# Dimitrinov74/Domain-Specific-Image-Compression

Hardware: AMD Instinct MI355X
Metric: 256x256 satellite patches encoded/s per GPU; bpp + MS-SSIM vs reference (higher is better)
Workload: dtype f32 (Winograd contractions as split-bf16 MFMA with fp32 accumulate); 1 GPU; batch=64/GPU 256x256x3 synthetic patches, modelv2 encode->decode (g_a,h_a,round,h_s,Student-t/Gaussian rate,g_s) + bpp + MS-SSIM[.3,.5,.2] on GPU + CDF tables and range coder (z,y strings) on GPU [BASELINE config 3]; global_batch=64, parallelism=per-image sharding x1, one all-reduce of 4 fp64, weights=synthetic seed 1 (checkpoints absent from the reference)

## Files before the change

### domain-specific-image-compression_amd/csrc/conv_wino_bf16.h

```cpp
#pragma once
#include <stdlib.h>

#include <type_traits>

#include "common.h"

#ifndef WB_PLANES
#define WB_PLANES 2
#endif
#ifndef WB_STAMP
#define WB_STAMP 0
#endif
#ifndef WB_ABL
#define WB_ABL 0
#endif
#ifndef WB_ADOUBLE
#define WB_ADOUBLE 0
#endif
#ifndef WB_HPRIO
#define WB_HPRIO 3
#endif
#ifndef WB_STAMP_TILE
#define WB_STAMP_TILE 8
#endif
// ... 19 lines not shown
  const float* beta;
  const float* gamma;
  float* out;
  int B, H, W, Cin, Cout, CoutP;
  int act;
  unsigned long long* ticket;
  int nphase;
  int64_t u_phase_bytes;
  int s2d_in, s2d;
  int tiles_x, tiles_y, ntiles;
  int nt_out;
  int ostride, ooff;
  int ksplit, kchunks;
  int64_t part_stride;
  int cm_in, cm_out;
};

constexpr int P = WB_PLANES;
constexpr int CK = 16;
constexpr int ROWB = CK * 2;
constexpr int POSB = 32 * ROWB;
constexpr int PLANEB = 16 * POSB;
constexpr int VBUFB = P * PLANEB;
constexpr int WP = 36;
constexpr int YOFF = 2 * VBUFB;
constexpr int YBYTES = 16 * 32 * WP * 4;
constexpr int SLOTOFF = YOFF + YBYTES;
constexpr int WINW = 18, WINH = 10;
constexpr int WINB = WINW * WINH * CK * 4;
constexpr int STAGEOFF = SLOTOFF + 64;
// ... 82 lines not shown
```

### domain-specific-image-compression_amd/csrc/conv_wino_bf16m.hip

```cpp
#include "conv_wino_bf16.h"

#ifndef WBM_STAMP
#define WBM_STAMP 0
#endif
#ifndef WBM_ABL
#define WBM_ABL 0
#endif

namespace dsic {
namespace wbm {

using wb::Args;
using wb::bf16_hi;
using wb::bf16_lo;
using wb::bf16x8;
using wb::cvt_pk_bf16;
using wb::floatx16;
using wb::floatx2;
using wb::floatx4;
using wb::intx4;
using wb::Tile;
using wb::uintx2;
using wb::uintx4;

// ... 2 lines not shown
constexpr int NTILE = 64;
constexpr int ROWB = CK * 2;
constexpr int POSB = NTILE * ROWB;
constexpr int PLANEB = 8 * POSB;
constexpr int VBUFB = P * PLANEB;
constexpr int XOFF = 2 * VBUFB;
constexpr int XBYTES = 8 * 4096;
constexpr int SLOTOFF = XOFF + XBYTES;
constexpr int WINW = 18, WINH = 18;
constexpr int WINITEMS = WINW * WINH * 4;
constexpr int WINB = WINITEMS * 16;
constexpr int NLOAD = (WINITEMS + 255) / 256;
constexpr int STAGEOFF = SLOTOFF + 64;
constexpr int NWIN = 3;
constexpr int STAMPOFF = STAGEOFF + NWIN * WINB;
constexpr int PARAMOFF = STAMPOFF + (WBM_STAMP ? 1024 : 0);
constexpr int LDS_TOTAL = PARAMOFF + 3 * 128 * 4;
constexpr int THREADS = 768;
constexpr int RING = 2;

static_assert(LDS_TOTAL <= 160 * 1024, "LDS budget");

#if WBM_STAMP
static __device__ long long wbm_stamps[256 * 256];
#define MSTAMP(w, i)                                                                                   \
  do {                                                                                                 \
    __builtin_amdgcn_sched_barrier(0);                                                                 \
    if (lane == 0 && wave == (w) && tile_count == 3 && (i) >= 0 && (i) < 128)                          \
      ((unsigned*)(lds_raw + STAMPOFF))[((w) == 0 ? 0 : 128) + (i)] = (unsigned)__builtin_amdgcn_s_memtime();   \
    __builtin_amdgcn_sched_barrier(0);                                                                 \
  } while (0)
#else
#define MSTAMP(w, i)
#endif

__device__ __forceinline__ int lane_now() {
  int l;
  asm volatile("v_mbcnt_lo_u32_b32 %0, -1, 0\n\tv_mbcnt_hi_u32_b32 %0, -1, %0" : "=v"(l));
  return l;
}

template <int MODE, int PASS, int PQ>
struct Steps {
  static constexpr unsigned value =
      PASS == 0 ? (PQ == 0 ? (MODE == 2 ? 0x4567u : 0x7654u) : (MODE == 2 ? 0x89ABu : 0xBA98u))
                : (PQ == 0 ? (MODE == 2 ? 0x0123u : 0x3210u) : (MODE == 2 ? 0xCDEFu : 0xFEDCu));
};
template <int MODE, int PASS, int PQ>
__device__ __forceinline__ constexpr int gpos(int s) {
  return (int)((Steps<MODE, PASS, PQ>::value >> (4 * s)) & 15u);
}
template <int PASS>
__device__ __forceinline__ constexpr int lpos_of(int g) {
  return PASS == 0 ? ((g >> 2) - 1) * 4 + (g & 3) : ((g >> 2) == 3 ? 4 : 0) + (g & 3);
}
template <int MODE, int PASS, int PQ>
__device__ __forceinline__ constexpr int step_of(int g) {
  for (int s = 0; s < 4; ++s)
    if (gpos<MODE, PASS, PQ>(s) == g) return s;
  return -1;
}

template <int MODE, bool NT_OUT>
__global__ __launch_bounds__(THREADS) void conv_wino_bf16m_kernel(const Args a) {
  extern __shared__ __attribute__((aligned(16))) unsigned char lds_raw[];
  float* const slots = (float*)(lds_raw + SLOTOFF);
  const int tid = threadIdx.x, lane = tid & 63;
  const int wave = __builtin_amdgcn_readfirstlane(tid >> 6);
  auto read_slot = [&](int s) {
    const intx4 v = *(const intx4*)(slots + 4 * s);
    Tile t;
    t.item = __builtin_amdgcn_readfirstlane(v[0]);
    t.tx = __builtin_amdgcn_readfirstlane(v[1]);
    t.ty = __builtin_amdgcn_readfirstlane(v[2]);
    t.n = __builtin_amdgcn_readfirstlane(v[3]);
    t.ks = 0;
    return t;
  };
  const int pshift = a.nphase == 4 ? 2 : 0;
  const int nchunks = a.Cin / CK;
  const int L = 2 * nchunks;
  int tile_count = 0;
  (void)tile_count;
  if (tid < 128) {
    float* const prm = (float*)(lds_raw + PARAMOFF);
    const bool cv = tid < a.Cout, gd = cv && (a.act == DSIC_ACT_GDN || a.act == DSIC_ACT_IGDN);
    prm[tid] = cv ? a.bias[tid] : 0.f;
    prm[128 + tid] = gd ? a.beta[tid] : 1.f;
    prm[256 + tid] = gd ? a.gamma[tid] : 0.f;
  }

  if (wave >= 8) {
    __builtin_amdgcn_s_setprio(3);
    const int ht = tid - 512;
    const int Cin = a.Cin;
    const int pt = ht >> 2, pq = ht & 3;
// ... 1 lines not shown
    const int vwrite = pt * ROWB + ((((pq >> 1) ^ ((pt >> 3) & 1))) << 4) + ((pq & 1) << 3);
    unsigned char* const vmine = lds_raw + vwrite;
    auto post = [&](int s, int item) {
      const int tile = item >> pshift;
      const int row = tile / a.tiles_x;
      const intx4 v = {item, tile - row * a.tiles_x, row % a.tiles_y, row / a.tiles_y};
      *(intx4*)(slots + 4 * s) = v;
    };
    const int pix_f = a.cm_in ? CK : Cin;
    const unsigned chunk_in_b = a.cm_in ? (unsigned)(a.H * a.W * CK * 4) : (unsigned)(CK * 4);
    struct WinAim {
      unsigned off[NLOAD];
      uintx4 rsrc;
    };
    WinAim am;
    const int hw = wave - 8;
    const unsigned lds_base = (unsigned)(unsigned long long)(__attribute__((address_space(3))) unsigned char*)lds_raw;
    auto aim = [&](WinAim& m, const Tile& t0) {
      Tile t = t0;
      if (WBM_ABL & 1) { t.n = 0; t.tx = 0; t.ty = 0; }
      const unsigned long long base = (unsigned long long)(a.in + (size_t)t.n * a.H * a.W * Cin);
      m.rsrc = uintx4{(unsigned)base, (unsigned)(base >> 32) & 0xFFFFu, (unsigned)(a.H * a.W * Cin * 4), 0x00020000u};
#pragma unroll
      for (int j = 0; j < NLOAD; ++j) {
        const int i = ht + 256 * j;
        const int pix = i >> 2, q = i & 3;
        const int wy = pix / WINW, wx = pix - wy * WINW;
        const int gy = t.ty * 16 - 1 + wy, gx = t.tx * 16 - 1 + wx;
        const bool ok = i < WINITEMS && gy >= 0 && gy < a.H && gx >= 0 && gx < a.W && !(WBM_ABL & 2);
        m.off[j] = ok ? (unsigned)(((gy * a.W + gx) * pix_f + 4 * q) * 4) : 0x80000000u;
      }
    };
    auto aim_nowhere = [&](WinAim& m) {
#pragma unroll
      for (int j = 0; j < NLOAD; ++j) m.off[j] = 0x80000000u;
    };
    auto dma = [&](int wbuf, int chunk) {
      const uintx4 rs = {(unsigned)__builtin_amdgcn_readfirstlane((int)am.rsrc[0]), (unsigned)__builtin_amdgcn_readfirstlane((int)am.rsrc[1]),
                         (unsigned)__builtin_amdgcn_readfirstlane((int)am.rsrc[2]), (unsigned)__builtin_amdgcn_readfirstlane((int)am.rsrc[3])};
      const unsigned soff = (unsigned)chunk * chunk_in_b;
#pragma unroll
      for (int j = 0; j < NLOAD; ++j) {
        const unsigned m0v = lds_base + (unsigned)(STAGEOFF + wbuf * WINB + 16 * (hw * 64 + 256 * j));
        if (j < NLOAD - 1 || ht < WINITEMS - 256 * (NLOAD - 1))
          asm volatile("s_mov_b32 m0, %0\n\ts_nop 0\n\tbuffer_load_dwordx4 %1, %2, %3 offen lds"
                       :: "s"(m0v), "v"(am.off[j]), "s"(rs), "s"(soff) : "memory");
      }
    };
    const bool last_piece = hw == 0;
    auto wait_all_but_newest = [&](int groups) {
      if (groups == 0) asm volatile("s_waitcnt vmcnt(0)" ::: "memory");
      else if (groups == 1) { if (last_piece) asm volatile("s_waitcnt vmcnt(6)" ::: "memory"); else asm volatile("s_waitcnt vmcnt(5)" ::: "memory"); }
      else { if (last_piece) asm volatile("s_waitcnt vmcnt(12)" ::: "memory"); else asm volatile("s_waitcnt vmcnt(10)" ::: "memory"); }
    };
    static_assert(NLOAD == 6, "the vmcnt immediates above count 6 (5) loads per window");
    const int patch0 = ((2 * pty) * WINW + 2 * ptx) * (CK * 4) + pq * 16;
    auto psub = [](floatx2 x, floatx2 y) {
      floatx2 r;
      asm("v_pk_add_f32 %0, %1, %2 neg_lo:[0,1] neg_hi:[0,1]" : "=v"(r) : "v"(x), "v"(y));
      return r;
    };
    auto sub4 = [&](floatx4 x, floatx4 y) {
      const floatx2 l = psub(floatx2{x[0], x[1]}, floatx2{y[0], y[1]}), h = psub(floatx2{x[2], x[3]}, floatx2{y[2], y[3]});
      return floatx4{l[0], l[1], h[0], h[1]};
    };
    auto split_store = [&](floatx4 v, unsigned char* dst) {
      const unsigned h0 = cvt_pk_bf16(v[0], v[1]), h1 = cvt_pk_bf16(v[2], v[3]);
      *(uintx2*)dst = uintx2{h0, h1};
      const floatx2 r01 = psub(floatx2{v[0], v[1]}, floatx2{bf16_lo(h0), bf16_hi(h0)});
      const floatx2 r23 = psub(floatx2{v[2], v[3]}, floatx2{bf16_lo(h1), bf16_hi(h1)});
// ... 3 lines not shown
      const unsigned char* src = lds_raw + STAGEOFF + wbuf * WINB + patch0;
      unsigned char* dst = vmine + vb * VBUFB;
      floatx4 xa[4], xb[4];
      bool a_live = true, b_live = true;
      if (!passB) {
#pragma unroll
        for (int k = 0; k < 4; ++k) {
          const floatx4 r1 = *(const floatx4*)(src + (1 * WINW + k) * (CK * 4));
          const floatx4 r2 = *(const floatx4*)(src + (2 * WINW + k) * (CK * 4));
          xa[k] = r1 + r2;
          xb[k] = sub4(r2, r1);
        }
      } else {
        a_live = zxi != 0u;
        b_live = zxi != 3u;
#pragma unroll
        for (int k = 0; k < 4; ++k) {
          const floatx4 r0 = *(const floatx4*)(src + (0 * WINW + k) * (CK * 4));
          const floatx4 r1 = *(const floatx4*)(src + (1 * WINW + k) * (CK * 4));
          const floatx4 r2 = *(const floatx4*)(src + (2 * WINW + k) * (CK * 4));
          const floatx4 r3 = *(const floatx4*)(src + (3 * WINW + k) * (CK * 4));
          xa[k] = sub4(r0, r2);
          xb[k] = sub4(r1, r3);
        }
      }
      if (a_live) {
        if (znu != 0) split_store(sub4(xa[0], xa[2]), dst + 0 * POSB);
        split_store(xa[1] + xa[2], dst + 1 * POSB);
        split_store(sub4(xa[2], xa[1]), dst + 2 * POSB);
        if (znu != 3) split_store(sub4(xa[1], xa[3]), dst + 3 * POSB);
      }
      if (b_live) {
        if (znu != 0) split_store(sub4(xb[0], xb[2]), dst + 4 * POSB);
        split_store(xb[1] + xb[2], dst + 5 * POSB);
        split_store(sub4(xb[2], xb[1]), dst + 6 * POSB);
        if (znu != 3) split_store(sub4(xb[1], xb[3]), dst + 7 * POSB);
      }
    };
    auto zero_of = [&](const Tile& t, int k, unsigned& zxi, unsigned& znu) {
      zxi = 4;
      znu = 4;
      if (MODE == 1) {
        const int blk = k / (nchunks >> 2);
        if (blk >> 1) zxi = 3;
        if (blk & 1) znu = 3;
      } else if (MODE == 2) {
        const int phase = t.item & 3;
        if (phase >> 1) zxi = 0;
        if (phase & 1) znu = 0;
      }
    };
    auto next_ticket = [&]() { return (int)(atomicAdd(a.ticket, 1ULL) + gridDim.x); };

    if (ht == 0) {
      post(0, (int)blockIdx.x);
      post(1, next_ticket());
    }
    __syncthreads();
    Tile cur = read_slot(0);
    int ticket_pre = a.ntiles;
    aim(am, cur);
    dma(0, 0);
    dma(1, 1);
    dma(2, 2);
    if (ht == 0 && read_slot(1).item < a.ntiles) ticket_pre = next_ticket();
    wait_all_but_newest(2);
    __syncthreads();
    {
      unsigned zxi, znu;
      zero_of(cur, 0, zxi, znu);
      commit(0, 0, false, zxi, znu);
    }
    wait_all_but_newest(1);
    __syncthreads();
    int wq = 1;
    int s_nxt = 1, s_wr = 2;
    while (cur.item < a.ntiles) {
      const Tile nxt = read_slot(s_nxt);
      const bool more = nxt.item < a.ntiles;
      tile_count++;
      auto phase = [&](int sg) {
        MSTAMP(8, 4 * sg);
        {
          const int k3 = sg + 3;
          if (k3 == L) {
            if (more) aim(am, nxt); else aim_nowhere(am);
          }
          const int k3w = k3 < L ? k3 : k3 - L;
          dma(wq >= 1 ? wq - 1 : 2, k3w < nchunks ? k3w : k3w - nchunks);
        }
        MSTAMP(8, 4 * sg + 1);
        {
          unsigned zxi, znu;
          const int tg = sg + 1;
          const bool passB = tg >= nchunks && tg < L;
          if (tg < L) zero_of(cur, passB ? tg - nchunks : tg, zxi, znu); else zero_of(nxt, 0, zxi, znu);
          commit(wq, tg & 1, passB, zxi, znu);
        }
        wq = wq == 2 ? 0 : wq + 1;
        wait_all_but_newest(1);
        MSTAMP(8, 4 * sg + 2);
        __syncthreads();
        MSTAMP(8, 4 * sg + 3);
      };
      if (ht == 0 && more) post(s_wr, ticket_pre);
      for (int sg = 0; sg < L; sg += 2) {
        phase(sg);
        phase(sg + 1);
        if (sg + 2 == nchunks) {
          __syncthreads();
          __syncthreads();
          __syncthreads();
          __syncthreads();
        }
      }
      if (ht == 0 && more && read_slot(s_wr).item < a.ntiles) ticket_pre = next_ticket();
      cur = nxt;
      const int s_old = s_nxt;
      s_nxt = s_wr;
      s_wr = s_old == 0 ? 2 : s_old - 1;
    }
#if WBM_STAMP
    if (wave == 8) {
      wbm_stamps[blockIdx.x * 256 + 128 + lane] = (long long)((unsigned*)(lds_raw + STAMPOFF))[128 + lane];
      wbm_stamps[blockIdx.x * 256 + 192 + lane] = (long long)((unsigned*)(lds_raw + STAMPOFF))[192 + lane];
    }
#endif
    if (ht == 0) {
      const unsigned long long done = atomicAdd(a.ticket + 1, 1ULL);
      if (done == (unsigned long long)gridDim.x - 1) {
        a.ticket[0] = 0ULL;
        a.ticket[1] = 0ULL;
      }
    }
    return;
  }

  const int h = lane >> 5, l31 = lane & 31;
  const int nt = wave & 3, pqw = wave >> 2;
  const bool nvalid = nt * 32 < a.CoutP;
// ... 50 lines not shown
  Tile cur = read_slot(0);
  const __amdgpu_buffer_rsrc_t urs = __builtin_amdgcn_make_buffer_rsrc(
      (void*)a.u, 0, (int)(16u * pos_b * (unsigned)a.nphase), 0x00020000);
  auto soff_item = [&](const Tile& t) { return (unsigned)(t.item & (a.nphase - 1)) * (unsigned)a.u_phase_bytes; };
  unsigned soff_phase = soff_item(cur);
  auto fetch = [&](bf16x8 (&dst)[P], unsigned so) {
#pragma unroll
    for (int q = 0; q < P; ++q)
      dst[q] = __builtin_bit_cast(bf16x8, __builtin_amdgcn_raw_buffer_load_b128(urs, ulane, so + (unsigned)q * plane_b, 0));
  };
#pragma unroll
  for (int f = 0; f < RING; ++f) fetch(Bq[f], soff_phase + (unsigned)gpos<MODE, 0, PQ>(f) * pos_b);
  int s_nxt = 1;
  while (cur.item < a.ntiles) {
    tile_count++;
    const Tile nxt = read_slot(s_nxt);
    const unsigned soff_phase_nxt = soff_item(nxt.item < a.ntiles ? nxt : cur);
    unsigned tzero_xi = 4, tzero_nu = 4;
    if (MODE == 2) {
      const int phase = cur.item & 3;
      if (phase >> 1) tzero_xi = 0;
      if (phase & 1) tzero_nu = 0;
    }
    auto chunk_body = [&](auto pass_tag, auto first_tag, int chunk) {
      constexpr int PASS = decltype(pass_tag)::value;
      constexpr bool FIRST = decltype(first_tag)::value;
      const bool last = chunk + 1 == nchunks;
      MSTAMP(0, 3 * (PASS * nchunks + chunk));
      unsigned zero_xi = tzero_xi, zero_nu = tzero_nu;
      if (MODE == 1) {
        const int blk = chunk / (nchunks >> 2);
        zero_xi = (blk >> 1) ? 3 : 4;
        zero_nu = (blk & 1) ? 3 : 4;
      }
      auto is_zero = [&](int s) {
        const int g = gpos<MODE, PASS, PQ>(s);
        return (unsigned)(g >> 2) == zero_xi || (unsigned)(g & 3) == zero_nu;
      };
      const unsigned char* vb = lds_raw + ((PASS * nchunks + chunk) & 1) * VBUFB + aread;
      auto vaddr = [&](int sub, int q) {
        return vb + lpos_of<PASS>(gpos<MODE, PASS, PQ>(sub >> 1)) * POSB + (sub & 1) * (32 * ROWB) + q * PLANEB;
      };
      bf16x8 Aq[P];
#pragma unroll
      for (int q = 0; q < P; ++q) Aq[q] = *(const bf16x8*)vaddr(0, q);
#pragma unroll
      for (int s = 0; s < 4; ++s) {
        const bool live = !ZSKIP || !is_zero(s);
// ... 11 lines not shown
#pragma unroll
            for (int e = 0; e < 16; ++e) acc[sub][e] = 0.f;
          }
          if (sub + 1 < 8) {
#pragma unroll
            for (int q = 0; q < P; ++q) Aq[q] = *(const bf16x8*)vaddr(sub + 1, q);
          }
        }
        {
          const int f = s + RING;
          const unsigned so = f < 4 ? soff_phase + (unsigned)gpos<MODE, PASS, PQ>(f) * pos_b + (unsigned)chunk * chunk_b
                                    : soff_phase + (unsigned)gpos<MODE, PASS, PQ>(f - 4) * pos_b + (unsigned)(chunk + 1) * chunk_b;
          if (f < 4 ? !(ZSKIP && is_zero(f)) : !last) fetch(Bq[s % RING], so);
        }
      }
      MSTAMP(0, 3 * (PASS * nchunks + chunk) + 1);
      __syncthreads();
      MSTAMP(0, 3 * (PASS * nchunks + chunk) + 2);
    };

    chunk_body(std::integral_constant<int, 0>{}, std::true_type{}, 0);
    for (int chunk = 1; chunk < nchunks; ++chunk) chunk_body(std::integral_constant<int, 0>{}, std::false_type{}, chunk);
    {
      constexpr int XI = 1 + PQ;
      constexpr int s0 = step_of<MODE, 0, PQ>(XI * 4 + 0), s1 = step_of<MODE, 0, PQ>(XI * 4 + 1);
      constexpr int s2 = step_of<MODE, 0, PQ>(XI * 4 + 2), s3 = step_of<MODE, 0, PQ>(XI * 4 + 3);
      floatx16 c0[2], c1[2];
#pragma unroll
      for (int m = 0; m < 2; ++m) {
        c0[m] = (acc[2 * s0 + m] + acc[2 * s1 + m]) + acc[2 * s2 + m];
        c1[m] = (acc[2 * s1 + m] - acc[2 * s2 + m]) - acc[2 * s3 + m];
      }
      constexpr int XB = PQ == 0 ? 0 : 3;
      constexpr int t0 = step_of<MODE, 1, PQ>(XB * 4 + 0), t1 = step_of<MODE, 1, PQ>(XB * 4 + 1);
      constexpr int t2 = step_of<MODE, 1, PQ>(XB * 4 + 2), t3 = step_of<MODE, 1, PQ>(XB * 4 + 3);
#pragma unroll
      for (int m = 0; m < 2; ++m) {
        xwrite(xa_mine, c0[m]);
        xwrite(xb_mine, c1[m]);
        MSTAMP(0, 122 + 2 * m);
        __syncthreads();
        MSTAMP(0, 123 + 2 * m);
        const floatx16 g0 = xread(xa_part), g1 = xread(xb_part);
        if (PQ == 0) {
          acc[2 * t0 + m] = c0[m] + g0;
          acc[2 * t3 + m] = -(c1[m] + g1);
        } else {
          acc[2 * t0 + m] = c0[m] - g0;
          acc[2 * t3 + m] = g1 - c1[m];
        }
#pragma unroll
        for (int e = 0; e < 16; ++e) {
          acc[2 * t1 + m][e] = 0.f;
          acc[2 * t2 + m][e] = 0.f;
        }
        __syncthreads();
      }
      MSTAMP(0, 126);
    }
#pragma unroll
    for (int f = 0; f < RING; ++f) fetch(Bq[f], soff_phase + (unsigned)gpos<MODE, 1, PQ>(f) * pos_b);
    for (int chunk = 0; chunk < nchunks; ++chunk) chunk_body(std::integral_constant<int, 1>{}, std::false_type{}, chunk);
    soff_phase = soff_phase_nxt;

    MSTAMP(0, 120);
    {
      const int phase = cur.item & (a.nphase - 1);
      const int ppy = phase >> 1, ppx = phase & 1;
      const int OH = a.nphase == 4 ? 2 * a.H : a.H, OW = a.nphase == 4 ? 2 * a.W : a.W;
      const __amdgpu_buffer_rsrc_t ors = __builtin_amdgcn_make_buffer_rsrc(
          (void*)(a.out + (size_t)cur.n * OH * OW * a.ostride + a.ooff), 0, (OH * OW * a.ostride - a.ooff) * 4, 0x00020000);
      const unsigned tbase =
          a.nphase == 4 ? (unsigned)(((32 * cur.ty + ppy) * OW + 32 * cur.tx + ppx) * PB)
          : a.s2d       ? (unsigned)(((8 * cur.ty) * (a.W >> 1) + 8 * cur.tx) * SX)
                        : (unsigned)((16 * cur.ty * a.W + 16 * cur.tx) * PB);
      constexpr int XB = PQ == 0 ? 0 : 3;
      constexpr int t0 = step_of<MODE, 1, PQ>(XB * 4 + 0), t1 = step_of<MODE, 1, PQ>(XB * 4 + 1);
      constexpr int t2 = step_of<MODE, 1, PQ>(XB * 4 + 2), t3 = step_of<MODE, 1, PQ>(XB * 4 + 3);
      const int ln = lane_now();
      float* const tw = (float*)(lds_raw + XOFF + wave * 4096) + ln + 96 * (ln >> 5);
// ... 36 lines not shown
        else if (a.act == DSIC_ACT_IGDN)
          emit(std::integral_constant<int, DSIC_ACT_IGDN>{}, m, j, y);
        else if (a.act == DSIC_ACT_RELU)
          emit(std::integral_constant<int, DSIC_ACT_RELU>{}, m, j, y);
        else
          emit(std::integral_constant<int, DSIC_ACT_NONE>{}, m, j, y);
      };
#pragma unroll
      for (int m = 0; m < 2; ++m) {
        const floatx16 y0 = (acc[2 * t0 + m] + acc[2 * t1 + m]) + acc[2 * t2 + m];
        const floatx16 y1 = (acc[2 * t1 + m] - acc[2 * t2 + m]) - acc[2 * t3 + m];
        emit_act(m, 0, PQ == 0 ? y0 : -y0);
        emit_act(m, 1, PQ == 0 ? y1 : -y1);
      }
    }
    MSTAMP(0, 121);
#pragma unroll
    for (int f = 0; f < RING; ++f) fetch(Bq[f], soff_phase + (unsigned)gpos<MODE, 0, PQ>(f) * pos_b);
    cur = nxt;
    s_nxt = s_nxt == 2 ? 0 : s_nxt + 1;
  }
#if WBM_STAMP
  if (wave == 0) {
    wbm_stamps[blockIdx.x * 256 + lane] = (long long)((unsigned*)(lds_raw + STAMPOFF))[lane];
    wbm_stamps[blockIdx.x * 256 + 64 + lane] = (long long)((unsigned*)(lds_raw + STAMPOFF))[64 + lane];
  }
#endif
  };
  if (pqw == 0)
    mfma_waves(std::integral_constant<int, 0>{});
  else
    mfma_waves(std::integral_constant<int, 1>{});
}

#undef xa_mine
#undef xa_part
#undef xb_mine
#undef xb_part

}
}

using namespace dsic;

extern "C" int dsic_wino_bf16_m64(int H, int W, int Cin, int nphase) {
  static int mode = -1;
  if (mode < 0) {
    const char* e = getenv("DSIC_WINO_M64");
    mode = e ? atoi(e) : 1;
  }
  if (!mode) return 0;
  if (H <= 0 || W <= 0 || H % 16 || W % 16 || Cin < 64 || Cin % 32) return 0;
  const int min_items = mode > 1 ? mode : 4;
  return (H / 16) * (W / 16) * nphase >= min_items;
}

int dsic_wbm_launch(wb::Args& a, hipStream_t st) {
  a.tiles_x = a.W / 16;
  a.tiles_y = a.H / 16;
  const int64_t nt = (int64_t)a.tiles_x * a.tiles_y * a.B * a.nphase;
  DSIC_REQUIRE(nt < ((int64_t)1 << 31), "conv_wino_bf16m: too many tiles");
  DSIC_REQUIRE((a.Cin / wbm::CK) % 2 == 0 && a.Cin / wbm::CK >= 4, "conv_wino_bf16m: Cin=%d", a.Cin);
  if (a.ostride <= 0) a.ostride = a.Cout;
  a.ntiles = (int)nt;
  a.ksplit = 1;
  a.nt_out = (int64_t)a.B * a.H * a.W * a.Cout * 4 * (a.nphase == 4 ? 4 : 1) > (300ll << 20);
  int dev = 0;
  if (hipGetDevice(&dev) != hipSuccess) dev = 0;
  if (dev < 0 || dev >= 64) dev = 0;
  static bool attr_set[64] = {};
  if (!attr_set[dev]) {
    const void* fns[6] = {(const void*)wbm::conv_wino_bf16m_kernel<0, false>, (const void*)wbm::conv_wino_bf16m_kernel<1, false>,
                          (const void*)wbm::conv_wino_bf16m_kernel<2, false>, (const void*)wbm::conv_wino_bf16m_kernel<0, true>,
                          (const void*)wbm::conv_wino_bf16m_kernel<1, true>,  (const void*)wbm::conv_wino_bf16m_kernel<2, true>};
    for (int i = 0; i < 6; ++i) {
      const hipError_t e = hipFuncSetAttribute(fns[i], hipFuncAttributeMaxDynamicSharedMemorySize, wbm::LDS_TOTAL);
      if (e != hipSuccess) {
        set_error("conv_wino_bf16m: hipFuncSetAttribute: %s", hipGetErrorString(e));
        return DSIC_EHIP;
      }
// ... 17 lines not shown
    else                                                                                                         \
      hipLaunchKernelGGL((wbm::conv_wino_bf16m_kernel<M, false>), dim3(grid), dim3(wbm::THREADS), wbm::LDS_TOTAL, st, a); \
  } while (0)
  if (a.s2d_in)
    WBM_LAUNCH(1);
  else if (a.nphase == 4)
    WBM_LAUNCH(2);
  else
    WBM_LAUNCH(0);
#undef WBM_LAUNCH
  return check_launch("conv_wino_bf16m");
}

#if WBM_STAMP
extern "C" int dsic_debug_wbm_stamps(long long* host_out) {
  return hipMemcpyFromSymbol(host_out, HIP_SYMBOL(wbm::wbm_stamps), sizeof(long long) * 256 * 256) == hipSuccess ? 0 : 2;
}
#endif
```

### domain-specific-image-compression_amd/lib.py

```python
from __future__ import annotations

import ctypes
import os
from ctypes import c_int, c_int64, c_void_p

HERE = os.path.dirname(os.path.abspath(__file__))
LIB_PATH = os.environ.get("DSIC_LIB") or os.path.join(HERE, "libdsic_hip.so")

DSIC_OK, DSIC_EINVAL, DSIC_EHIP = 0, 1, 2
ACT_NONE, ACT_GDN, ACT_IGDN, ACT_RELU = 0, 1, 2, 3

_P = c_void_p
SIGNATURES = {
    "dsic_last_error": (ctypes.c_char_p, []),
    "dsic_abi_version": (c_int, []),
    "dsic_split_bf16": (c_int, []),
    "dsic_set_split_bf16": (c_int, [c_int]),
    "dsic_packed_conv_weight_floats": (c_int64, [c_int, c_int, c_int]),
    "dsic_pack_conv_weight": (c_int, [_P, _P, c_int, c_int, c_int, _P]),
    "dsic_pack_convT_weight": (c_int, [_P, _P, c_int, c_int, _P]),
    "dsic_convT_image_weight_floats": (c_int64, [c_int]),
    "dsic_pack_convT_image_weight": (c_int, [_P, _P, c_int, c_int, _P]),
    "dsic_image_to_nhwc8": (c_int, [_P, _P, c_int, c_int, c_int, c_int, _P]),
    "dsic_nhwc_to_nchw": (c_int, [_P, _P, c_int, c_int, c_int, c_int, _P]),
# ... 5 lines not shown
    "dsic_wino_weight_floats": (c_int64, [c_int, c_int]),
    "dsic_pack_wino_weight": (c_int, [_P, _P, c_int, c_int, _P]),
    "dsic_conv3x3_wino_nhwc": (c_int, [_P, _P, _P, _P, _P, _P, c_int, c_int, c_int, c_int, c_int, c_int, c_int, c_int,
                                       _P, _P]),
    "dsic_pack_wino_s2_weight": (c_int, [_P, _P, c_int, c_int, _P]),
    "dsic_pack_wino_convT_weight": (c_int, [_P, _P, c_int, c_int, _P]),
    "dsic_conv_transpose2d_wino_nhwc": (c_int, [_P, _P, _P, _P, _P, _P, c_int, c_int, c_int, c_int, c_int, c_int, _P,
                                                _P]),
    "dsic_wino_bf16_planes": (c_int, []),
    "dsic_wino_bf16_weight_bytes": (c_int64, [c_int, c_int]),
    "dsic_split_wino_weight_bf16": (c_int, [_P, _P, c_int, c_int, c_int, _P]),
    "dsic_conv3x3_wino_bf16_nhwc": (c_int, [_P, _P, _P, _P, _P, _P, c_int, c_int, c_int, c_int, c_int, c_int, c_int,
                                            c_int, c_int, c_int, _P, _P]),
    "dsic_wino_bf16_ksplit": (c_int, [c_int, c_int, c_int]),
    "dsic_wino_bf16_m64": (c_int, [c_int, c_int, c_int, c_int]),
    "dsic_conv3x3_wino_bf16_splitk_nhwc": (c_int, [_P, _P, _P, _P, _P, _P, c_int, c_int, c_int, c_int, c_int, c_int,
                                                   c_int, c_int, c_int, c_int, c_int, _P, _P, _P]),
    "dsic_conv_transpose2d_wino_bf16_nhwc": (c_int, [_P, _P, _P, _P, _P, _P, c_int, c_int, c_int, c_int, c_int, c_int,
                                                     _P, _P]),
    "dsic_conv_transpose2d_wino_bf16_layout": (c_int, [_P, _P, _P, _P, _P, _P, c_int, c_int, c_int, c_int, c_int,
                                                       c_int, c_int, c_int, _P, _P]),
    "dsic_conv_first_nchw": (c_int, [_P, _P, _P, _P, _P, _P, c_int, c_int, c_int, c_int, c_int, c_int, c_int, _P]),
    "dsic_conv_first_u8hwc": (c_int, [_P, _P, _P, _P, _P, _P, c_int, c_int, c_int, c_int, c_int, c_int, c_int, _P]),
    "dsic_image_u8hwc_to_f32nchw": (c_int, [_P, _P, c_int, c_int, c_int, c_int, _P]),
    "dsic_conv_transpose2d_nhwc": (c_int, [_P, _P, _P, _P, _P, _P, c_int, c_int, c_int, c_int,
                                           c_int, c_int, _P]),
    "dsic_conv_transpose2d_image": (c_int, [_P, _P, _P, _P, c_int, c_int, c_int, c_int, c_int, _P]),
    "dsic_hyper_params": (c_int, [_P] * 13 + [c_int, c_int, c_int, c_int, ctypes.c_float,
                                     ctypes.c_float, _P]),
    "dsic_rate_workspace_doubles": (c_int64, [c_int]),
# ... 88 lines not shown
```

### include/dsic_hip.h

```cpp
#ifndef DSIC_HIP_H
#define DSIC_HIP_H

#include <stdint.h>

#ifdef __cplusplus
extern "C" {
#endif

#define DSIC_OK 0
#define DSIC_EINVAL 1
#define DSIC_EHIP 2

#define DSIC_ACT_NONE 0
#define DSIC_ACT_GDN 1
#define DSIC_ACT_IGDN 2
#define DSIC_ACT_RELU 3
#define DSIC_LAYOUT_CM16 2

const char* dsic_last_error(void);
int dsic_abi_version(void);

int dsic_split_bf16(void);
int dsic_set_split_bf16(int on);

// ... 46 lines not shown
                                    const float* gamma, float* out, int B,
                                    int H, int W, int Cin, int Cout, int act,
                                    void* ticket, void* stream);

int dsic_wino_bf16_planes(void);
int64_t dsic_wino_bf16_weight_bytes(int Cout, int Cin);
int dsic_split_wino_weight_bf16(const float* u_f32, void* dst, int Cout, int Cin,
                                int nphase, void* stream);
int dsic_conv3x3_wino_bf16_nhwc(const float* in, const void* u_planes,
                                const float* bias, const float* beta,
                                const float* gamma, float* out, int B, int H, int W,
                                int Cin, int Cout, int act, int s2d_out, int s2d_in,
                                int out_cstride, int out_coff, void* ticket, void* stream);
int dsic_wino_bf16_ksplit(int H, int W, int Cin);
int dsic_wino_bf16_m64(int H, int W, int Cin, int nphase);
int dsic_conv3x3_wino_bf16_splitk_nhwc(const float* in, const void* u_planes,
                                       const float* bias, const float* beta,
                                       const float* gamma, float* out, int B, int H, int W,
                                       int Cin, int Cout, int act, int s2d_out, int s2d_in,
                                       int out_cstride, int out_coff, int ksplit,
                                       float* partials, void* ticket, void* stream);
int dsic_conv_transpose2d_wino_bf16_nhwc(const float* in, const void* u_planes4,
                                         const float* bias, const float* beta,
                                         const float* gamma, float* out, int B,
                                         int H, int W, int Cin, int Cout, int act,
                                         void* ticket, void* stream);
int dsic_conv_transpose2d_wino_bf16_layout(const float* in, const void* u_planes4,
                                           const float* bias, const float* beta,
                                           const float* gamma, float* out, int B,
                                           int H, int W, int Cin, int Cout, int act,
// ... 164 lines not shown
```

Before: 11180 images/s.

## Pair half-dead pass-B chunks in the m64 Winograd kernel to skip zero work

When a pass-B chunk has a structurally dead xi row (the zero-padded phases in modes 1 and 2), two such chunks are now packed into one window buffer. Each half loads only the live rows, and a new commit and MFMA body handles both at once, which shortens pass B from nchunks to roughly nchunks/2 steps for those tiles. The aim is to remove wasted DMA, commit and barrier work on zero regions. It also makes the regular commit skip loading rows whose outputs are dead. In exchange the scheduling logic becomes considerably more complex, and the change adds a host-side schedule-checking API and an environment toggle that defaults to on.

```diff
diff --git a/domain-specific-image-compression_amd/csrc/conv_wino_bf16.h b/domain-specific-image-compression_amd/csrc/conv_wino_bf16.h
--- a/domain-specific-image-compression_amd/csrc/conv_wino_bf16.h
+++ b/domain-specific-image-compression_amd/csrc/conv_wino_bf16.h
@@ -57,6 +57,7 @@
   int ksplit, kchunks;
   int64_t part_stride;
   int cm_in, cm_out;
+  int pair_b;
 };
 
 constexpr int P = WB_PLANES;
diff --git a/domain-specific-image-compression_amd/csrc/conv_wino_bf16m.hip b/domain-specific-image-compression_amd/csrc/conv_wino_bf16m.hip
--- a/domain-specific-image-compression_amd/csrc/conv_wino_bf16m.hip
+++ b/domain-specific-image-compression_amd/csrc/conv_wino_bf16m.hip
@@ -1,7 +1,11 @@
 #include "conv_wino_bf16.h"
+#include "conv_wino_pair.h"
 
 #ifndef WBM_STAMP
 #define WBM_STAMP 0
+#endif
+#ifndef WBM_STAMP_C0
+#define WBM_STAMP_C0 0
 #endif
 #ifndef WBM_ABL
 #define WBM_ABL 0
@@ -40,51 +44,38 @@
 constexpr int STAGEOFF = SLOTOFF + 64;
 constexpr int NWIN = 3;
 constexpr int STAMPOFF = STAGEOFF + NWIN * WINB;
-constexpr int PARAMOFF = STAMPOFF + (WBM_STAMP ? 1024 : 0);
+constexpr int PARAMOFF = STAMPOFF + (WBM_STAMP ? 1536 : 0);
 constexpr int LDS_TOTAL = PARAMOFF + 3 * 128 * 4;
 constexpr int THREADS = 768;
 constexpr int RING = 2;
+constexpr int PAIRITEMS = 9 * WINW * 4;
+constexpr int PAIRHALFB = PAIRITEMS * 16;
 
 static_assert(LDS_TOTAL <= 160 * 1024, "LDS budget");
+static_assert(2 * PAIRITEMS == WINITEMS, "a paired window fills one window buffer, piece for piece");
 
 #if WBM_STAMP
-static __device__ long long wbm_stamps[256 * 256];
+static __device__ long long wbm_stamps[256 * 384];
 #define MSTAMP(w, i)                                                                                   \
   do {                                                                                                 \
     __builtin_amdgcn_sched_barrier(0);                                                                 \
     if (lane == 0 && wave == (w) && tile_count == 3 && (i) >= 0 && (i) < 128)                          \
-      ((unsigned*)(lds_raw + STAMPOFF))[((w) == 0 ? 0 : 128) + (i)] = (unsigned)__builtin_amdgcn_s_memtime();   \
+      ((unsigned*)(lds_raw + STAMPOFF))[((w) == 0 ? 0 : (w) == 8 ? 128 : 256) + (i)] = (unsigned)__builtin_amdgcn_s_memtime();   \
     __builtin_amdgcn_sched_barrier(0);                                                                 \
+  } while (0)
+#define MSTAMPC(w, sigma, k, PER)                                                                      \
+  do {                                                                                                 \
+    if ((sigma) >= WBM_STAMP_C0 && (sigma) < WBM_STAMP_C0 + 32) MSTAMP(w, (PER) * ((sigma) - WBM_STAMP_C0) + (k)); \
   } while (0)
 #else
 #define MSTAMP(w, i)
+#define MSTAMPC(w, sigma, k, PER)
 #endif
 
 __device__ __forceinline__ int lane_now() {
   int l;
   asm volatile("v_mbcnt_lo_u32_b32 %0, -1, 0\n\tv_mbcnt_hi_u32_b32 %0, -1, %0" : "=v"(l));
   return l;
-}
-
-template <int MODE, int PASS, int PQ>
-struct Steps {
-  static constexpr unsigned value =
-      PASS == 0 ? (PQ == 0 ? (MODE == 2 ? 0x4567u : 0x7654u) : (MODE == 2 ? 0x89ABu : 0xBA98u))
-                : (PQ == 0 ? (MODE == 2 ? 0x0123u : 0x3210u) : (MODE == 2 ? 0xCDEFu : 0xFEDCu));
-};
-template <int MODE, int PASS, int PQ>
-__device__ __forceinline__ constexpr int gpos(int s) {
-  return (int)((Steps<MODE, PASS, PQ>::value >> (4 * s)) & 15u);
-}
-template <int PASS>
-__device__ __forceinline__ constexpr int lpos_of(int g) {
-  return PASS == 0 ? ((g >> 2) - 1) * 4 + (g & 3) : ((g >> 2) == 3 ? 4 : 0) + (g & 3);
-}
-template <int MODE, int PASS, int PQ>
-__device__ __forceinline__ constexpr int step_of(int g) {
-  for (int s = 0; s < 4; ++s)
-    if (gpos<MODE, PASS, PQ>(s) == g) return s;
-  return -1;
 }
 
 template <int MODE, bool NT_OUT>
@@ -105,7 +96,8 @@
   };
   const int pshift = a.nphase == 4 ? 2 : 0;
   const int nchunks = a.Cin / CK;
-  const int L = 2 * nchunks;
+  constexpr bool PAIR = MODE != 0;
+  auto pfirst_of = [&](const Tile& t) { return PAIR ? pair_first(MODE, nchunks, t.item & 3, a.pair_b != 0) : nchunks; };
   int tile_count = 0;
   (void)tile_count;
   if (tid < 128) {
@@ -137,6 +129,7 @@
       uintx4 rsrc;
     };
     WinAim am;
+    unsigned off2[NLOAD];
     const int hw = wave - 8;
     const unsigned lds_base = (unsigned)(unsigned long long)(__attribute__((address_space(3))) unsigned char*)lds_raw;
     auto aim = [&](WinAim& m, const Tile& t0) {
@@ -158,7 +151,22 @@
 #pragma unroll
       for (int j = 0; j < NLOAD; ++j) m.off[j] = 0x80000000u;
     };
-    auto dma = [&](int wbuf, int chunk) {
+    auto aim2 = [&](const Tile& t0) {
+      Tile t = t0;
+      if (WBM_ABL & 1) { t.n = 0; t.tx = 0; t.ty = 0; }
+#pragma unroll
+      for (int j = 0; j < NLOAD; ++j) {
+        const int i = ht + 256 * j;
+        const int half = i >= PAIRITEMS ? 1 : 0;
+        const int ii = i - half * PAIRITEMS;
+        const int pix = ii >> 2, q = ii & 3;
+        const int r = pix / WINW, wx = pix - r * WINW;
+        const int gy = t.ty * 16 - 1 + pair_window_row(MODE, r), gx = t.tx * 16 - 1 + wx;
+        const bool ok = i < WINITEMS && gy >= 0 && gy < a.H && gx >= 0 && gx < a.W && !(WBM_ABL & 2);
+        off2[j] = ok ? (unsigned)(((gy * a.W + gx) * pix_f + 4 * q) * 4) + (unsigned)half * chunk_in_b : 0x80000000u;
+      }
+    };
+    auto dma = [&](int wbuf, int chunk, const unsigned (&off)[NLOAD]) {
       const uintx4 rs = {(unsigned)__builtin_amdgcn_readfirstlane((int)am.rsrc[0]), (unsigned)__builtin_amdgcn_readfirstlane((int)am.rsrc[1]),
                          (unsigned)__builtin_amdgcn_readfirstlane((int)am.rsrc[2]), (unsigned)__builtin_amdgcn_readfirstlane((int)am.rsrc[3])};
       const unsigned soff = (unsigned)chunk * chunk_in_b;
@@ -167,7 +175,7 @@
         const unsigned m0v = lds_base + (unsigned)(STAGEOFF + wbuf * WINB + 16 * (hw * 64 + 256 * j));
         if (j < NLOAD - 1 || ht < WINITEMS - 256 * (NLOAD - 1))
           asm volatile("s_mov_b32 m0, %0\n\ts_nop 0\n\tbuffer_load_dwordx4 %1, %2, %3 offen lds"
-                       :: "s"(m0v), "v"(am.off[j]), "s"(rs), "s"(soff) : "memory");
+                       :: "s"(m0v), "v"(off[j]), "s"(rs), "s"(soff) : "memory");
       }
     };
     const bool last_piece = hw == 0;
@@ -176,7 +184,7 @@
       else if (groups == 1) { if (last_piece) asm volatile("s_waitcnt vmcnt(6)" ::: "memory"); else asm volatile("s_waitcnt vmcnt(5)" ::: "memory"); }
       else { if (last_piece) asm volatile("s_waitcnt vmcnt(12)" ::: "memory"); else asm volatile("s_waitcnt vmcnt(10)" ::: "memory"); }
     };
-    static_assert(NLOAD == 6, "the vmcnt immediates above count 6 (5) loads per window");
+    static_assert(NLOAD == 6 && 2 * PAIRITEMS == WINITEMS, "the vmcnt immediates above count 6 (5) loads per window, whole or paired");
     const int patch0 = ((2 * pty) * WINW + 2 * ptx) * (CK * 4) + pq * 16;
     auto psub = [](floatx2 x, floatx2 y) {
       floatx2 r;
@@ -210,14 +218,28 @@
       } else {
         a_live = zxi != 0u;
         b_live = zxi != 3u;
-#pragma unroll
-        for (int k = 0; k < 4; ++k) {
-          const floatx4 r0 = *(const floatx4*)(src + (0 * WINW + k) * (CK * 4));
-          const floatx4 r1 = *(const floatx4*)(src + (1 * WINW + k) * (CK * 4));
-          const floatx4 r2 = *(const floatx4*)(src + (2 * WINW + k) * (CK * 4));
-          const floatx4 r3 = *(const floatx4*)(src + (3 * WINW + k) * (CK * 4));
-          xa[k] = sub4(r0, r2);
-          xb[k] = sub4(r1, r3);
+        floatx4 r0[4], r1[4], r2[4], r3[4];
+        if (a_live) {
+#pragma unroll
+          for (int k = 0; k < 4; ++k) {
+            r0[k] = *(const floatx4*)(src + (0 * WINW + k) * (CK * 4));
+            r2[k] = *(const floatx4*)(src + (2 * WINW + k) * (CK * 4));
+          }
+        }
+        if (b_live) {
+#pragma unroll
+          for (int k = 0; k < 4; ++k) {
+            r1[k] = *(const floatx4*)(src + (1 * WINW + k) * (CK * 4));
+            r3[k] = *(const floatx4*)(src + (3 * WINW + k) * (CK * 4));
+          }
+        }
+        if (a_live) {
+#pragma unroll
+          for (int k = 0; k < 4; ++k) xa[k] = sub4(r0[k], r2[k]);
+        }
+        if (b_live) {
+#pragma unroll
+          for (int k = 0; k < 4; ++k) xb[k] = sub4(r1[k], r3[k]);
         }
       }
       if (a_live) {
@@ -234,16 +256,32 @@
       }
     };
     auto zero_of = [&](const Tile& t, int k, unsigned& zxi, unsigned& znu) {
-      zxi = 4;
-      znu = 4;
-      if (MODE == 1) {
-        const int blk = k / (nchunks >> 2);
-        if (blk >> 1) zxi = 3;
-        if (blk & 1) znu = 3;
-      } else if (MODE == 2) {
-        const int phase = t.item & 3;
-        if (phase >> 1) zxi = 0;
-        if (phase & 1) znu = 0;
+      zxi = zero_xi_of(MODE, nchunks, t.item & 3, k);
+      znu = zero_nu_of(MODE, nchunks, t.item & 3, k);
+    };
+    auto commit_pair = [&](int wbuf, int vb, const Tile& t, int c) {
+      const unsigned char* src = lds_raw + STAGEOFF + wbuf * WINB + (pty * WINW + 2 * ptx) * (CK * 4) + pq * 16;
+      unsigned char* dst = vmine + vb * VBUFB;
+      floatx4 ra[2][4], rb[2][4];
+#pragma unroll
+      for (int hf = 0; hf < 2; ++hf) {
+#pragma unroll
+        for (int k = 0; k < 4; ++k) {
+          ra[hf][k] = *(const floatx4*)(src + hf * PAIRHALFB + k * (CK * 4));
+          rb[hf][k] = *(const floatx4*)(src + hf * PAIRHALFB + (WINW + k) * (CK * 4));
+        }
+      }
+#pragma unroll
+      for (int hf = 0; hf < 2; ++hf) {
+        unsigned zxi, znu;
+        zero_of(t, c + hf, zxi, znu);
+        floatx4 x[4];
+#pragma unroll
+        for (int k = 0; k < 4; ++k) x[k] = sub4(ra[hf][k], rb[hf][k]);
+        if (znu != 0) split_store(sub4(x[0], x[2]), dst + pair_commit_slot(MODE, hf, 0) * POSB);
+        split_store(x[1] + x[2], dst + pair_commit_slot(MODE, hf, 1) * POSB);
+        split_store(sub4(x[2], x[1]), dst + pair_commit_slot(MODE, hf, 2) * POSB);
+        if (znu != 3) split_store(sub4(x[1], x[3]), dst + pair_commit_slot(MODE, hf, 3) * POSB);
       }
     };
     auto next_ticket = [&]() { return (int)(atomicAdd(a.ticket, 1ULL) + gridDim.x); };
@@ -256,9 +294,11 @@
     Tile cur = read_slot(0);
     int ticket_pre = a.ntiles;
     aim(am, cur);
-    dma(0, 0);
-    dma(1, 1);
-    dma(2, 2);
+    const bool pair_on = PAIR && a.pair_b != 0;
+    if (pair_on && pfirst_of(cur) < nchunks) aim2(cur);
+    dma(0, 0, am.off);
+    dma(1, 1, am.off);
+    dma(2, 2, am.off);
     if (ht == 0 && read_slot(1).item < a.ntiles) ticket_pre = next_ticket();
     wait_all_but_newest(2);
     __syncthreads();
@@ -275,29 +315,40 @@
       const Tile nxt = read_slot(s_nxt);
       const bool more = nxt.item < a.ntiles;
       tile_count++;
+      const int pfirst = pfirst_of(cur);
+      const int L = nchunks + pass_b_len(nchunks, pfirst);
       auto phase = [&](int sg) {
-        MSTAMP(8, 4 * sg);
+        MSTAMPC(8, sg, 0, 4);
         {
           const int k3 = sg + 3;
           if (k3 == L) {
             if (more) aim(am, nxt); else aim_nowhere(am);
+            if (pair_on && more && pfirst_of(nxt) < nchunks) aim2(nxt);
           }
-          const int k3w = k3 < L ? k3 : k3 - L;
-          dma(wq >= 1 ? wq - 1 : 2, k3w < nchunks ? k3w : k3w - nchunks);
-        }
-        MSTAMP(8, 4 * sg + 1);
+          const int wb3 = wq >= 1 ? wq - 1 : 2;
+          const int jb = k3 - nchunks;
+          if (PAIR && k3 < L && jb >= pfirst)
+            dma(wb3, pass_b_chunk(jb, pfirst), off2);
+          else
+            dma(wb3, k3 < nchunks ? k3 : k3 < L ? jb : k3 - L, am.off);
+        }
+        MSTAMPC(8, sg, 1, 4);
         {
           unsigned zxi, znu;
           const int tg = sg + 1;
           const bool passB = tg >= nchunks && tg < L;
-          if (tg < L) zero_of(cur, passB ? tg - nchunks : tg, zxi, znu); else zero_of(nxt, 0, zxi, znu);
-          commit(wq, tg & 1, passB, zxi, znu);
+          if (PAIR && passB && tg - nchunks >= pfirst) {
+            commit_pair(wq, tg & 1, cur, pass_b_chunk(tg - nchunks, pfirst));
+          } else {
+            if (tg < L) zero_of(cur, passB ? tg - nchunks : tg, zxi, znu); else zero_of(nxt, 0, zxi, znu);
+            commit(wq, tg & 1, passB, zxi, znu);
+          }
         }
         wq = wq == 2 ? 0 : wq + 1;
         wait_all_but_newest(1);
-        MSTAMP(8, 4 * sg + 2);
+        MSTAMPC(8, sg, 2, 4);
         __syncthreads();
-        MSTAMP(8, 4 * sg + 3);
+        MSTAMPC(8, sg, 3, 4);
       };
       if (ht == 0 && more) post(s_wr, ticket_pre);
       for (int sg = 0; sg < L; sg += 2) {
@@ -318,8 +369,8 @@
     }
 #if WBM_STAMP
     if (wave == 8) {
-      wbm_stamps[blockIdx.x * 256 + 128 + lane] = (long long)((unsigned*)(lds_raw + STAMPOFF))[128 + lane];
-      wbm_stamps[blockIdx.x * 256 + 192 + lane] = (long long)((unsigned*)(lds_raw + STAMPOFF))[192 + lane];
+      wbm_stamps[blockIdx.x * 384 + 128 + lane] = (long long)((unsigned*)(lds_raw + STAMPOFF))[128 + lane];
+      wbm_stamps[blockIdx.x * 384 + 192 + lane] = (long long)((unsigned*)(lds_raw + STAMPOFF))[192 + lane];
     }
 #endif
     if (ht == 0) {
@@ -400,6 +451,9 @@
   int s_nxt = 1;
   while (cur.item < a.ntiles) {
     tile_count++;
+#if WBM_STAMP
+    if (lane == 0 && wave == 4 * PQ && tile_count == 3) ((unsigned*)(lds_raw + STAMPOFF))[(PQ ? 256 : 0) + 127] = (unsigned)cur.item;
+#endif
     const Tile nxt = read_slot(s_nxt);
     const unsigned soff_phase_nxt = soff_item(nxt.item < a.ntiles ? nxt : cur);
     unsigned tzero_xi = 4, tzero_nu = 4;
@@ -412,12 +466,11 @@
       constexpr int PASS = decltype(pass_tag)::value;
       constexpr bool FIRST = decltype(first_tag)::value;
       const bool last = chunk + 1 == nchunks;
-      MSTAMP(0, 3 * (PASS * nchunks + chunk));
+      MSTAMPC(4 * PQ, PASS * nchunks + chunk, 0, 3);
       unsigned zero_xi = tzero_xi, zero_nu = tzero_nu;
       if (MODE == 1) {
-        const int blk = chunk / (nchunks >> 2);
-        zero_xi = (blk >> 1) ? 3 : 4;
-        zero_nu = (blk & 1) ? 3 : 4;
+        zero_xi = zero_xi_of(MODE, nchunks, 0, chunk);
+        zero_nu = zero_nu_of(MODE, nchunks, 0, chunk);
       }
       auto is_zero = [&](int s) {
         const int g = gpos<MODE, PASS, PQ>(s);
@@ -459,9 +512,51 @@
           if (f < 4 ? !(ZSKIP && is_zero(f)) : !last) fetch(Bq[s % RING], so);
         }
       }
-      MSTAMP(0, 3 * (PASS * nchunks + chunk) + 1);
+      MSTAMPC(4 * PQ, PASS * nchunks + chunk, 1, 3);
       __syncthreads();
-      MSTAMP(0, 3 * (PASS * nchunks + chunk) + 2);
+      MSTAMPC(4 * PQ, PASS * nchunks + chunk, 2, 3);
+    };
+    auto pair_body = [&](int j, int chunk) {
+      const bool last = chunk + 2 == nchunks;
+      MSTAMPC(4 * PQ, nchunks + j, 0, 3);
+      auto is_zero = [&](int s) {
+        return (unsigned)(pair_gpos<MODE, PQ>(s) & 3) == zero_nu_of(MODE, nchunks, cur.item & 3, chunk + pair_half(s));
+      };
+      const unsigned char* vb = lds_raw + (j & 1) * VBUFB + aread;
+      auto vaddr = [&](int sub, int q) {
+        return vb + pair_vslot<MODE, PQ>(sub >> 1) * POSB + (sub & 1) * (32 * ROWB) + q * PLANEB;
+      };
+      bf16x8 Aq[P];
+#pragma unroll
+      for (int q = 0; q < P; ++q) Aq[q] = *(const bf16x8*)vaddr(0, q);
+#pragma unroll
+      for (int s = 0; s < 8; ++s) {
+        const bool live = !is_zero(s);
+#pragma unroll
+        for (int m = 0; m < 2; ++m) {
+          const int sub = 2 * s + m, ai = 2 * pair_acc(s) + m;
+          if (live) {
+            floatx16 c = acc[ai];
+            c = __builtin_amdgcn_mfma_f32_32x32x16_bf16(Aq[0], Bq[s % RING][1], c, 0, 0, 0);
+            c = __builtin_amdgcn_mfma_f32_32x32x16_bf16(Aq[1], Bq[s % RING][0], c, 0, 0, 0);
+            c = __builtin_amdgcn_mfma_f32_32x32x16_bf16(Aq[0], Bq[s % RING][0], c, 0, 0, 0);
+            acc[ai] = c;
+          }
+          if (sub + 1 < 16) {
+#pragma unroll
+            for (int q = 0; q < P; ++q) Aq[q] = *(const bf16x8*)vaddr(sub + 1, q);
+          }
+        }
+        {
+          const int f = s + RING;
+          const unsigned so = soff_phase + (unsigned)pair_gpos<MODE, PQ>(f & 7) * pos_b +
+                              (unsigned)(chunk + (f < 8 ? pair_half(f) : 2)) * chunk_b;
+          if (f < 8 ? !is_zero(f) : !last) fetch(Bq[s % RING], so);
+        }
+      }
+      MSTAMPC(4 * PQ, nchunks + j, 1, 3);
+      __syncthreads();
+      MSTAMPC(4 * PQ, nchunks + j, 2, 3);
     };
 
     chunk_body(std::integral_constant<int, 0>{}, std::true_type{}, 0);
@@ -483,9 +578,9 @@
       for (int m = 0; m < 2; ++m) {
         xwrite(xa_mine, c0[m]);
         xwrite(xb_mine, c1[m]);
-        MSTAMP(0, 122 + 2 * m);
+        MSTAMP(4 * PQ, 122 + 2 * m);
         __syncthreads();
-        MSTAMP(0, 123 + 2 * m);
+        MSTAMP(4 * PQ, 123 + 2 * m);
         const floatx16 g0 = xread(xa_part), g1 = xread(xb_part);
         if (PQ == 0) {
           acc[2 * t0 + m] = c0[m] + g0;
@@ -501,14 +596,27 @@
         }
         __syncthreads();
       }
-      MSTAMP(0, 126);
+      MSTAMP(4 * PQ, 126);
     }
 #pragma unroll
     for (int f = 0; f < RING; ++f) fetch(Bq[f], soff_phase + (unsigned)gpos<MODE, 1, PQ>(f) * pos_b);
-    for (int chunk = 0; chunk < nchunks; ++chunk) chunk_body(std::integral_constant<int, 1>{}, std::false_type{}, chunk);
+    const int pfirst = pfirst_of(cur);
+    for (int chunk = 0; chunk < pfirst; ++chunk) chunk_body(std::integral_constant<int, 1>{}, std::false_type{}, chunk);
+    if constexpr (PAIR) {
+      for (int j = pfirst; j < pass_b_len(nchunks, pfirst); ++j) {
+        if constexpr (PQ == pair_owner(MODE)) {
+          pair_body(j, pass_b_chunk(j, pfirst));
+        } else {
+          MSTAMPC(4 * PQ, nchunks + j, 0, 3);
+          MSTAMPC(4 * PQ, nchunks + j, 1, 3);
+          __syncthreads();
+          MSTAMPC(4 * PQ, nchunks + j, 2, 3);
+        }
+      }
+    }
     soff_phase = soff_phase_nxt;
 
-    MSTAMP(0, 120);
+    MSTAMP(4 * PQ, 120);
     {
       const int phase = cur.item & (a.nphase - 1);
       const int ppy = phase >> 1, ppx = phase & 1;
@@ -575,16 +683,17 @@
         emit_act(m, 1, PQ == 0 ? y1 : -y1);
       }
     }
-    MSTAMP(0, 121);
+    MSTAMP(4 * PQ, 121);
 #pragma unroll
     for (int f = 0; f < RING; ++f) fetch(Bq[f], soff_phase + (unsigned)gpos<MODE, 0, PQ>(f) * pos_b);
     cur = nxt;
     s_nxt = s_nxt == 2 ? 0 : s_nxt + 1;
   }
 #if WBM_STAMP
-  if (wave == 0) {
-    wbm_stamps[blockIdx.x * 256 + lane] = (long long)((unsigned*)(lds_raw + STAMPOFF))[lane];
-    wbm_stamps[blockIdx.x * 256 + 64 + lane] = (long long)((unsigned*)(lds_raw + STAMPOFF))[64 + lane];
+  if (wave == 0 || wave == 4) {
+    unsigned* const st = (unsigned*)(lds_raw + STAMPOFF) + (wave == 0 ? 0 : 256);
+    wbm_stamps[blockIdx.x * 384 + (wave == 0 ? 0 : 256) + lane] = (long long)st[lane];
+    wbm_stamps[blockIdx.x * 384 + (wave == 0 ? 0 : 256) + 64 + lane] = (long long)st[64 + lane];
   }
 #endif
   };
@@ -614,6 +723,73 @@
   if (H <= 0 || W <= 0 || H % 16 || W % 16 || Cin < 64 || Cin % 32) return 0;
   const int min_items = mode > 1 ? mode : 4;
   return (H / 16) * (W / 16) * nphase >= min_items;
+}
+
+static int wbm_pair_mode() {
+  static int mode = -1;
+  if (mode < 0) {
+    const char* e = getenv("DSIC_WINO_PAIR");
+    mode = e ? (atoi(e) != 0) : 1;
+  }
+  return mode;
+}
+static int wbm_pair_override = -1;
+extern "C" int dsic_wino_pair_chunks(int on) {
+  const int was = wbm_pair_override >= 0 ? wbm_pair_override : wbm_pair_mode();
+  if (on >= 0) wbm_pair_override = on != 0;
+  return was;
+}
+
+namespace {
+template <int MODE, int PQ>
+int pass_b_sequence(int nchunks, int phase, bool paired, int acc, int* out, int cap) {
+  using namespace dsic::wbm;
+  int n = 0;
+  auto put = [&](int chunk, int g) {
+    if (n < cap) {
+      out[2 * n] = chunk;
+      out[2 * n + 1] = g;
+    }
+    ++n;
+  };
+  auto live = [&](int chunk, int g) {
+    return (unsigned)(g >> 2) != zero_xi_of(MODE, nchunks, phase, chunk) && (unsigned)(g & 3) != zero_nu_of(MODE, nchunks, phase, chunk);
+  };
+  const int pfirst = MODE == 0 ? nchunks : pair_first(MODE, nchunks, phase, paired);
+  for (int j = 0; j < pass_b_len(nchunks, pfirst); ++j) {
+    const int c = pass_b_chunk(j, pfirst);
+    if (j < pfirst) {
+      for (int s = 0; s < 4; ++s)
+        if (s == acc && live(c, gpos<MODE, 1, PQ>(s))) put(c, gpos<MODE, 1, PQ>(s));
+    } else if (PQ == pair_owner(MODE)) {
+      for (int s = 0; s < 8; ++s) {
+        const int g = pair_gpos<MODE, PQ>(s), cc = c + pair_half(s);
+        if (pair_vslot<MODE, PQ>(s) != pair_commit_slot(MODE, pair_half(s), g & 3) || (g >> 2) != pair_live_xi(MODE)) return -2;
+        if (pair_acc(s) == acc && live(cc, g)) put(cc, g);
+      }
+    } else {
+      for (int h = 0; h < 2; ++h)
+        for (int s = 0; s < 4; ++s)
+          if (live(c + h, gpos<MODE, 1, PQ>(s))) return -3;
+    }
+  }
+  return n;
+}
+}
+extern "C" int dsic_wino_pair_schedule(int mode, int nchunks, int phase, int paired, int pq, int acc, int* out, int cap) {
+  if (mode < 0 || mode > 2 || nchunks < 4 || nchunks % 2 || phase < 0 || phase > 3 || pq < 0 || pq > 1 || acc < 0 || acc > 3 ||
+      (cap > 0 && !out))
+    return -1;
+#define WBM_SEQ(M, Q) pass_b_sequence<M, Q>(nchunks, phase, paired != 0, acc, out, cap)
+  switch (mode * 2 + pq) {
+    case 0: return WBM_SEQ(0, 0);
+    case 1: return WBM_SEQ(0, 1);
+    case 2: return WBM_SEQ(1, 0);
+    case 3: return WBM_SEQ(1, 1);
+    case 4: return WBM_SEQ(2, 0);
+    default: return WBM_SEQ(2, 1);
+  }
+#undef WBM_SEQ
 }
 
 int dsic_wbm_launch(wb::Args& a, hipStream_t st) {
@@ -625,6 +801,7 @@
   if (a.ostride <= 0) a.ostride = a.Cout;
   a.ntiles = (int)nt;
   a.ksplit = 1;
+  a.pair_b = dsic_wino_pair_chunks(-1);
   a.nt_out = (int64_t)a.B * a.H * a.W * a.Cout * 4 * (a.nphase == 4 ? 4 : 1) > (300ll << 20);
   int dev = 0;
   if (hipGetDevice(&dev) != hipSuccess) dev = 0;
@@ -672,6 +849,6 @@
 
 #if WBM_STAMP
 extern "C" int dsic_debug_wbm_stamps(long long* host_out) {
-  return hipMemcpyFromSymbol(host_out, HIP_SYMBOL(wbm::wbm_stamps), sizeof(long long) * 256 * 256) == hipSuccess ? 0 : 2;
+  return hipMemcpyFromSymbol(host_out, HIP_SYMBOL(wbm::wbm_stamps), sizeof(long long) * 256 * 384) == hipSuccess ? 0 : 2;
 }
 #endif
diff --git a/domain-specific-image-compression_amd/csrc/conv_wino_pair.h b/domain-specific-image-compression_amd/csrc/conv_wino_pair.h
--- /dev/null
+++ b/domain-specific-image-compression_amd/csrc/conv_wino_pair.h
@@ -0,0 +1,67 @@
+#pragma once
+
+#if defined(__HIPCC__)
+#define WBM_HD __host__ __device__ __forceinline__
+#else
+#define WBM_HD inline
+#endif
+
+namespace dsic {
+namespace wbm {
+
+template <int MODE, int PASS, int PQ>
+struct Steps {
+  static constexpr unsigned value =
+      PASS == 0 ? (PQ == 0 ? (MODE == 2 ? 0x4567u : 0x7654u) : (MODE == 2 ? 0x89ABu : 0xBA98u))
+                : (PQ == 0 ? (MODE == 2 ? 0x0123u : 0x3210u) : (MODE == 2 ? 0xCDEFu : 0xFEDCu));
+};
+template <int MODE, int PASS, int PQ>
+WBM_HD constexpr int gpos(int s) {
+  return (int)((Steps<MODE, PASS, PQ>::value >> (4 * s)) & 15u);
+}
+template <int PASS>
+WBM_HD constexpr int lpos_of(int g) {
+  return PASS == 0 ? ((g >> 2) - 1) * 4 + (g & 3) : ((g >> 2) == 3 ? 4 : 0) + (g & 3);
+}
+template <int MODE, int PASS, int PQ>
+WBM_HD constexpr int step_of(int g) {
+  for (int s = 0; s < 4; ++s)
+    if (gpos<MODE, PASS, PQ>(s) == g) return s;
+  return -1;
+}
+
+WBM_HD constexpr int pair_dead_xi(int mode) { return mode == 2 ? 0 : 3; }
+WBM_HD constexpr int pair_live_xi(int mode) { return mode == 2 ? 3 : 0; }
+WBM_HD constexpr int pair_owner(int mode) { return mode == 2 ? 1 : 0; }
+WBM_HD constexpr int pair_first(int mode, int nchunks, int phase, bool on) {
+  if (!on) return nchunks;
+  if (mode == 1) return nchunks % 8 == 0 ? nchunks / 2 : nchunks;
+  if (mode == 2) return ((phase >> 1) & 1) && nchunks % 4 == 0 ? 0 : nchunks;
+  return nchunks;
+}
+WBM_HD constexpr int pass_b_len(int nchunks, int pfirst) { return pfirst + (nchunks - pfirst) / 2; }
+WBM_HD constexpr int pass_b_chunk(int j, int pfirst) { return j < pfirst ? j : pfirst + 2 * (j - pfirst); }
+WBM_HD constexpr unsigned zero_xi_of(int mode, int nchunks, int phase, int k) {
+  return mode == 1 ? (k >= 2 * (nchunks >> 2) ? 3u : 4u) : mode == 2 ? (((phase >> 1) & 1) ? 0u : 4u) : 4u;
+}
+WBM_HD constexpr unsigned zero_nu_of(int mode, int nchunks, int phase, int k) {
+  return mode == 1 ? (((k >= (nchunks >> 2) && k < 2 * (nchunks >> 2)) || k >= 3 * (nchunks >> 2)) ? 3u : 4u)
+                   : mode == 2 ? ((phase & 1) ? 0u : 4u) : 4u;
+}
+WBM_HD constexpr int pair_half(int s) { return s >> 2; }
+WBM_HD constexpr int pair_acc(int s) { return s & 3; }
+template <int MODE, int PQ>
+WBM_HD constexpr int pair_gpos(int s) {
+  return gpos<MODE, 1, PQ>(s & 3);
+}
+template <int MODE, int PQ>
+WBM_HD constexpr int pair_vslot(int s) {
+  return lpos_of<1>(pair_gpos<MODE, PQ>(s)) ^ (pair_half(s) << 2);
+}
+WBM_HD constexpr int pair_commit_slot(int mode, int half, int nu) {
+  return ((pair_live_xi(mode) == 3 ? 4 : 0) ^ (half << 2)) + nu;
+}
+WBM_HD constexpr int pair_window_row(int mode, int r) { return 2 * r + (pair_live_xi(mode) == 3 ? 1 : 0); }
+
+}
+}
diff --git a/domain-specific-image-compression_amd/lib.py b/domain-specific-image-compression_amd/lib.py
--- a/domain-specific-image-compression_amd/lib.py
+++ b/domain-specific-image-compression_amd/lib.py
@@ -43,6 +43,8 @@
                                             c_int, c_int, c_int, _P, _P]),
     "dsic_wino_bf16_ksplit": (c_int, [c_int, c_int, c_int]),
     "dsic_wino_bf16_m64": (c_int, [c_int, c_int, c_int, c_int]),
+    "dsic_wino_pair_chunks": (c_int, [c_int]),
+    "dsic_wino_pair_schedule": (c_int, [c_int, c_int, c_int, c_int, c_int, c_int, _P, c_int]),
     "dsic_conv3x3_wino_bf16_splitk_nhwc": (c_int, [_P, _P, _P, _P, _P, _P, c_int, c_int, c_int, c_int, c_int, c_int,
                                                    c_int, c_int, c_int, c_int, c_int, _P, _P, _P]),
     "dsic_conv_transpose2d_wino_bf16_nhwc": (c_int, [_P, _P, _P, _P, _P, _P, c_int, c_int, c_int, c_int, c_int, c_int,
diff --git a/include/dsic_hip.h b/include/dsic_hip.h
--- a/include/dsic_hip.h
+++ b/include/dsic_hip.h
@@ -84,6 +84,8 @@
                                 int out_cstride, int out_coff, void* ticket, void* stream);
 int dsic_wino_bf16_ksplit(int H, int W, int Cin);
 int dsic_wino_bf16_m64(int H, int W, int Cin, int nphase);
+int dsic_wino_pair_chunks(int on);
+int dsic_wino_pair_schedule(int mode, int nchunks, int phase, int paired, int pq, int acc, int* out, int cap);
 int dsic_conv3x3_wino_bf16_splitk_nhwc(const float* in, const void* u_planes,
                                        const float* bias, const float* beta,
                                        const float* gamma, float* out, int B, int H, int W,
```

After: 11360 images/s, median of 6. 1.6% higher.
